# jkulhanek/viewformer

Hardware: AMD Instinct MI355X
Metric: novel views/sec (encode->AR transformer->decode), 128px 6-ctx (higher is better)
Workload: dtype bf16

## Files before the change

include/vf_hip.h:

```cpp
#ifndef VF_HIP_H
#define VF_HIP_H

#include <stddef.h>
#include <stdint.h>

#ifdef __cplusplus
extern "C" {
#endif

#define VF_OK 0
#define VF_ERR_BAD_ARG (-1)
#define VF_ERR_UNSUPPORTED (-2)

int vf_abi_version(void);
size_t vf_sizeof_igemm_args(void);
size_t vf_sizeof_pack_desc(void);
const char* vf_build_arch(void);
int vf_build_flags(void);
const char* vf_build_flag_name(int i);
enum { VF_SEL_ATTN_DMA = 0,
       VF_SEL_GEMM_G256 = 1,
       VF_SEL_LN_BWD_TWO_ROWS = 2,
       VF_SEL_ATTN_Q32 = 3,
       VF_SEL_CONV_X3H_K32 = 4,
// ... 135 lines not shown
                          float* max_logit, void* stream);
int vf_lmhead_score_bf16(const void* h, int h_bf16, int64_t ldh, const void* w_packed, int64_t M, int K, int N, const int32_t* target,
                         int64_t* idx, float* max_logit, float* lse, float* target_logit, float* entropy, void* stream);
int vf_logits_score_f32(const float* logits, int64_t rows, int N, int64_t ld, const int32_t* target, int64_t* idx, float* max_logit,
                        float* lse, float* target_logit, float* entropy, void* stream);
int vf_score_views_f32(const float* target_logit, const float* lse, const float* max_logit, const int64_t* idx, const int32_t* target,
                       int64_t views, int L, float* token_log_prob, float* confidence, float* log_likelihood, float* accuracy, void* stream);
int vf_match_views_f32(const float* logits, int64_t ld, const float* lse, const int64_t* idx, const int32_t* codes, int64_t codes_scene_stride,
                       int64_t B, int64_t M, int64_t P, int L, int V, float* log_likelihood, float* accuracy, void* stream);
int vf_sample_rows_f32(const float* logits, int64_t rows, int N, int64_t ld, float temperature, int top_k, float top_p, uint32_t seed,
                       const int64_t* row_id, int S, int64_t* idx, float* logp, int32_t* kept, float* thr, void* stream);
int vf_sample_views_f32(const float* logp, int64_t views, int L, int S, float* log_likelihood, void* stream);
uint32_t vf_crc32c(const void* data, size_t n, uint32_t crc);
int vf_postprocess_u8(const float* x, uint8_t* out, int64_t n, void* stream);
int vf_resize_u8(const uint8_t* src, uint8_t* dst, int n_img, int Hin, int Win, int Hout, int Wout, int C, int bilinear, void* stream);
size_t vf_image_metrics_workspace_bytes(int n_img, int H, int W, int C);
int vf_image_metrics_u8(const uint8_t* a, const uint8_t* b, int n_img, int H, int W, int C, int64_t* sums, double* ssim, void* workspace,
                        void* stream);
size_t vf_camera_knn_workspace_bytes(int64_t N, int Q, int k);
int vf_camera_knn_f32(const float* db, int64_t N, const float* queries, int Q, int k, float pos_weight, int32_t* idx, float* dist,
                      void* workspace, void* stream);
int vf_codebook_dist_table_f32(const float* E, int D, int K, int64_t ldE, float* table, void* stream);
size_t vf_code_knn_workspace_bytes(int64_t N, int Q, int k);
int vf_code_knn_f32(const int32_t* db, int64_t N, int64_t ld_db, const int32_t* queries, int Q, int64_t ld_q, int t, const float* table,
                    int K, int window, const int32_t* exclude, int k, int32_t* idx, float* dist, void* workspace, void* stream);
int vf_pose_tail_f32(const float* x, int64_t ldx, const float* W, const float* b, float position_multiplier, int64_t views, int L, int K,
                     float* raw, float* tokens, float* cameras, void* stream);

size_t vf_gemm_bf16_packed_elems(int K, int N);
int vf_gemm_bf16_pack(const float* src, void* dst, int K, int N, int64_t sk, int64_t sn, int batch,
                      int64_t src_bstride, void* stream);
typedef struct vf_pack_desc {
    const float* src;
    void* dst;
    int32_t K, N;
    int64_t sk, sn;
} vf_pack_desc;
int vf_gemm_bf16_pack_multi(const vf_pack_desc* descs_device, int n, void* stream);
int vf_gemm_bf16(const vf_igemm_args* args , void* stream);
size_t vf_conv3_bf16_packed_elems(int Cin, int Cout);
int vf_conv3_bf16_pack(const float* w_oihw, void* dst, int Cin, int Cout, void* stream);
int vf_conv3_halo_bf16(const vf_igemm_args* args , void* stream);

int vf_conv3_halo_gn_slots(int Hout, int Wout);
size_t vf_conv3_x6_packed_elems(int Cin, int Cout);
int vf_conv3_x6_pack(const float* w_oihw, void* dst, int Cin, int Cout, void* stream);
int vf_conv3_halo_x6(const vf_igemm_args* args , void* stream);
size_t vf_conv3_x3h_packed_elems(int Cin, int Cout);
int vf_conv3_x3h_pack(const float* w_oihw, void* dst, int Cin, int Cout, void* stream);
int vf_conv3_halo_x3h(const vf_igemm_args* args , void* stream);
size_t vf_gemm_x3h_packed_elems(int K, int N);
int vf_gemm_x3h_pack(const float* src, void* dst, int K, int N, int64_t sk, int64_t sn, void* stream);
int vf_gemm_x3h(const vf_igemm_args* args , void* stream);
size_t vf_gemm_x6_packed_elems(int K, int N);
int vf_gemm_x6_pack(const float* src, void* dst, int K, int N, int64_t sk, int64_t sn, void* stream);
int vf_gemm_x6(const vf_igemm_args* args , void* stream);
int vf_sum_slabs_f32(const float* slabs, int nslabs, int64_t stride, int64_t n, float* dst, int accumulate, void* stream);

int vf_vq_ema_accumulate_f32(const float* z, const int64_t* idx, int64_t M, int D, int Kc, float* counts, float* embed_sum,
                             void* stream);
int vf_vq_ema_update_f32(const float* counts, const float* embed_sum, float* cluster_size_hidden, float* dw_hidden,
                         float* embeddings, int D, int Kc, float decay, float eps, float corr, void* stream);

int vf_gather_transpose_f32(const float* src, float* dst, int n_img, int Hin, int Win, int C, int Hout, int Wout, int stride, int oy,
                            int ox, int64_t ld_dst, void* stream);
size_t vf_conv3_wgrad_x6_rows(int Cin);
int vf_conv3_wgrad_x6(const float* x, const void* dy_packed, float* slabs, int n_img, int Hin, int Win, int Cin, int Hout, int Wout,
                      int Cout, int mode, int splits, void* stream);
int vf_upsample2_bwd_f32(const float* du, float* dx, int n_img, int H, int W, int C, void* stream);
size_t vf_groupnorm_bwd_workspace_bytes(int n_img, int HW, int C, int groups);
int vf_groupnorm_bwd_f32(const float* x, const float* da, const float* mean_c, const float* scale_c, const float* gamma,
                         const float* beta, float* dx, float* chan_sums, int n_img, int HW, int C, int groups, float eps, int swish,
                         int accumulate, void* ws, void* stream);
int vf_softmax_rows_bwd_f32(const float* p, float* dp, int64_t rows, int n, float scale, void* stream);
int vf_l1_loss_partials(int64_t n);
int vf_l1_loss_f32(const float* x, const float* y, float* dy, float* part, int64_t n, float grad_weight, void* stream);

int vf_lpips_scaling_f32(const float* x, float* y, int64_t npix, const float* shift3, const float* scale3, int backward, void* stream);
int vf_relu_f32(float* x, int64_t n, void* stream);
int vf_relu_bwd_f32(float* dy, const float* y, int64_t n, void* stream);
int vf_maxpool2_f32(const float* x, float* y, int n_img, int Hout, int Wout, int C, void* stream);
int vf_maxpool2_bwd_f32(const float* x, const float* dy, float* dx, int n_img, int Hout, int Wout, int C, void* stream);
int vf_lpips_head_blocks(int HW);
int vf_lpips_head_f32(const float* f0, const float* f1, const float* w, float* part, int n_img, int HW, int C, void* stream);
int vf_lpips_head_bwd_f32(const float* f0, const float* f1, const float* w, float* df1, int64_t npix, int C, float gscale,
                          int accumulate, void* stream);

int vf_attn_blockcausal_lse_f32(const float* q, const float* k, const float* v, float* out, float* lse,
                                int B, int H, int T, int L, int ldq, int ldk, int ldv, int ldo,
                                float scale, int skip_masked, int twin_view, float drop_rate, uint32_t drop_seed,
                                uint32_t drop_site, uint32_t drop_plane0, void* stream);
int vf_attn_bwd_prep_f32(const float* dout, const float* out, float* D, int B, int H, int T, int lddo, int ldo, void* stream);
int vf_attn_bwd_f32(const float* q, const float* k, const float* v, const float* dout, const float* lse, const float* D,
                    float* dq, float* dk, float* dv, int B, int H, int T, int L, int ldq, int ldk, int ldv, int lddo,
                    int lddq, int lddk, int lddv, float scale, int twin_view, float drop_rate, uint32_t drop_seed,
                    uint32_t drop_site, uint32_t drop_plane0, void* stream);
int vf_gemm_tn_bf16(const void* x_bf16, int ldx, const void* dy, int dy_is_bf16, int ldy, int M, int K, int N, int splits, float* w_slabs,
                    float* b_slabs, int64_t slab_stride, void* stream);
int vf_attn_blockcausal_bf16_lse(const void* q, const void* k, const void* v, void* out, float* lse, int B, int H, int T, int L,
                                 int ldq, int ldk, int ldv, int ldo, float scale, int twin_view, float drop_rate, uint32_t drop_seed,
                                 uint32_t drop_site, uint32_t drop_plane0, void* stream);
int vf_attn_bwd_prep_bf16(const void* dout, const void* out, float* D, int B, int H, int T, int lddo, int ldo, void* stream);
int vf_attn_bwd_bf16(const void* q, const void* k, const void* v, const void* dout, const float* lse, const float* D, void* dq, void* dk,
                     void* dv, int out_bf16 , int B, int H, int T, int L,
                     int ldq, int ldk, int ldv, int lddo, int lddq, int lddk, int lddv, float scale, int twin_view, float drop_rate,
                     uint32_t drop_seed, uint32_t drop_site, uint32_t drop_plane0, void* stream);
// ... 60 lines not shown
```

viewformer_amd/_lib.py:

```python
import ctypes
import os
from ctypes import c_int, c_int32, c_int64, c_float, c_void_p, c_size_t, c_char_p, POINTER

HERE = os.path.dirname(os.path.abspath(__file__))
LIB_PATH = os.environ.get('VF_HIP_LIB') or os.path.join(HERE, 'libvf_hip.so')


class VfIgemmArgs(ctypes.Structure):
    _fields_ = [
        ('x', c_void_p), ('w_packed', c_void_p), ('bias', c_void_p), ('res', c_void_p), ('out', c_void_p),
        ('pro_mean', c_void_p), ('pro_scale', c_void_p), ('pro_beta', c_void_p),
        ('pro_swish', c_int32), ('pro_rows_per_img', c_int32), ('mode', c_int32), ('epilogue', c_int32),
        ('M', c_int32), ('Cin', c_int32), ('Cout', c_int32),
        ('Hin', c_int32), ('Win', c_int32), ('Hout', c_int32), ('Wout', c_int32),
        ('lda', c_int32), ('ldc', c_int32), ('ldr', c_int32), ('batch', c_int32),
        ('stride_x', c_int64), ('stride_w', c_int64), ('stride_out', c_int64), ('stride_res', c_int64),
        ('gn_part', c_void_p), ('gn_slots', c_int32), ('reserved0', c_int32),
        ('out_aux', c_void_p),
        ('drop_rate', c_float), ('drop_seed', ctypes.c_uint32), ('drop_site', ctypes.c_uint32), ('drop_row0', c_int32),
    ]


SEL_ATTN_DMA, SEL_GEMM_G256, SEL_LN_BWD_TWO_ROWS, SEL_ATTN_Q32 = 0, 1, 2, 3
SEL_CONV_X3H_K32 = 4
# ... 76 lines not shown
    'vf_attn_blockcausal_lse_f32': (c_int, [P, P, P, P, P, c_int, c_int, c_int, c_int, c_int, c_int, c_int, c_int,
                                            c_float, c_int, c_int, c_float, ctypes.c_uint32, ctypes.c_uint32, ctypes.c_uint32, P]),
    'vf_dropout_add_f32': (c_int, [P, P, P, c_int64, c_int, c_int64, c_float, ctypes.c_uint32, ctypes.c_uint32, P]),
    'vf_attn_bwd_prep_f32': (c_int, [P, P, P, c_int, c_int, c_int, c_int, c_int, P]),
    'vf_attn_bwd_f32': (c_int, [P, P, P, P, P, P, P, P, P, c_int, c_int, c_int, c_int, c_int, c_int, c_int, c_int, c_int,
                                c_int, c_int, c_float, c_int, c_float, ctypes.c_uint32, ctypes.c_uint32, ctypes.c_uint32, P]),
    'vf_gemm_tn_bf16': (c_int, [P, c_int, P, c_int, c_int, c_int, c_int, c_int, c_int, P, P, c_int64, P]),
    'vf_attn_blockcausal_bf16_lse': (c_int, [P, P, P, P, P, c_int, c_int, c_int, c_int, c_int, c_int, c_int, c_int, c_float, c_int,
                                             c_float, ctypes.c_uint32, ctypes.c_uint32, ctypes.c_uint32, P]),
    'vf_attn_bwd_prep_bf16': (c_int, [P, P, P, c_int, c_int, c_int, c_int, c_int, P]),
    'vf_attn_bwd_bf16': (c_int, [P, P, P, P, P, P, P, P, P, c_int, c_int, c_int, c_int, c_int, c_int, c_int, c_int, c_int, c_int, c_int, c_int,
                                 c_float, c_int, c_float, ctypes.c_uint32, ctypes.c_uint32, ctypes.c_uint32, P]),
    'vf_attn_spatial_f32': (c_int, [P, P, c_int, c_int, c_int, c_int64, c_int64, c_float, P]),
    'vf_attn_spatial_x3h': (c_int, [P, P, c_int, c_int, c_int, c_int64, c_int64, c_float, P]),
    'vf_softmax_rows_f32': (c_int, [P, c_int64, c_int, c_float, P]),
    'vf_layernorm_f32': (c_int, [P, P, P, P, c_int64, c_int, c_float, P]),
    'vf_layernorm_bf16out_f32': (c_int, [P, P, P, P, c_int64, c_int, c_float, P]),
    'vf_embed_sum_f32': (c_int, [P, P, P, P, P, c_int64, c_int, c_int, c_int, P]),
    'vf_dense_small_k_gelu_f32': (c_int, [P, P, P, P, c_int64, c_int, c_int, c_int, P]),
    'vf_lmhead_argmax_bf16': (c_int, [P, c_int, c_int64, P, c_int64, c_int, c_int, P, P, P]),
    'vf_lmhead_score_bf16': (c_int, [P, c_int, c_int64, P, c_int64, c_int, c_int, P, P, P, P, P, P, P]),
    'vf_logits_score_f32': (c_int, [P, c_int64, c_int, c_int64, P, P, P, P, P, P, P]),
    'vf_score_views_f32': (c_int, [P, P, P, P, P, c_int64, c_int, P, P, P, P, P]),
    'vf_match_views_f32': (c_int, [P, c_int64, P, P, P, c_int64, c_int64, c_int64, c_int64, c_int, c_int, P, P, P]),
    'vf_sample_rows_f32': (c_int, [P, c_int64, c_int, c_int64, c_float, c_int, c_float, ctypes.c_uint32, P, c_int, P, P, P, P, P]),
    'vf_sample_views_f32': (c_int, [P, c_int64, c_int, c_int, P, P]),
    'vf_argmax_rows_f32': (c_int, [P, c_int64, c_int, c_int, P, P]),
    'vf_postprocess_u8': (c_int, [P, P, c_int64, P]),
    'vf_resize_u8': (c_int, [P, P, c_int, c_int, c_int, c_int, c_int, c_int, c_int, P]),
    'vf_image_metrics_workspace_bytes': (c_size_t, [c_int, c_int, c_int, c_int]),
    'vf_image_metrics_u8': (c_int, [P, P, c_int, c_int, c_int, c_int, P, P, P, P]),
    'vf_camera_knn_workspace_bytes': (c_size_t, [c_int64, c_int, c_int]),
    'vf_camera_knn_f32': (c_int, [P, c_int64, P, c_int, c_int, c_float, P, P, P, P]),
    'vf_codebook_dist_table_f32': (c_int, [P, c_int, c_int, c_int64, P, P]),
    'vf_code_knn_workspace_bytes': (c_size_t, [c_int64, c_int, c_int]),
    'vf_code_knn_f32': (c_int, [P, c_int64, c_int64, P, c_int, c_int64, c_int, P, c_int, c_int, P, c_int, P, P, P, P]),
    'vf_pose_tail_f32': (c_int, [P, c_int64, P, P, c_float, c_int64, c_int, c_int, P, P, P, P]),
    'vf_gemm_bf16_packed_elems': (c_size_t, [c_int, c_int]),
    'vf_gemm_bf16_pack': (c_int, [P, P, c_int, c_int, c_int64, c_int64, c_int, c_int64, P]),
    'vf_gemm_bf16_pack_multi': (c_int, [P, c_int, P]),
    'vf_gemm_bf16': (c_int, [POINTER(VfIgemmArgs), P]),
    'vf_conv3_bf16_packed_elems': (c_size_t, [c_int, c_int]),
    'vf_conv3_bf16_pack': (c_int, [P, P, c_int, c_int, P]),
    'vf_conv3_halo_bf16': (c_int, [POINTER(VfIgemmArgs), P]),
    'vf_conv3_x6_packed_elems': (c_size_t, [c_int, c_int]),
    'vf_conv3_x6_pack': (c_int, [P, P, c_int, c_int, P]),
    'vf_conv3_halo_x6': (c_int, [POINTER(VfIgemmArgs), P]),
    'vf_conv3_x3h_packed_elems': (c_size_t, [c_int, c_int]),
    'vf_conv3_x3h_pack': (c_int, [P, P, c_int, c_int, P]),
    'vf_conv3_halo_x3h': (c_int, [POINTER(VfIgemmArgs), P]),
    'vf_gemm_x3h_packed_elems': (c_size_t, [c_int, c_int]),
    'vf_gemm_x3h_pack': (c_int, [P, P, c_int, c_int, c_int64, c_int64, P]),
    'vf_gemm_x3h': (c_int, [POINTER(VfIgemmArgs), P]),
    'vf_gemm_x6_packed_elems': (c_size_t, [c_int, c_int]),
    'vf_gemm_x6_pack': (c_int, [P, P, c_int, c_int, c_int64, c_int64, P]),
    'vf_gemm_x6': (c_int, [POINTER(VfIgemmArgs), P]),
    'vf_sum_slabs_f32': (c_int, [P, c_int, c_int64, c_int64, P, c_int, P]),
    'vf_transpose_f32': (c_int, [P, P, c_int, c_int, c_int64, c_int64, c_int, c_int64, c_int64, P]),
    'vf_transpose_bf16_f32': (c_int, [P, P, c_int, c_int, c_int64, c_int64, c_int, c_int64, c_int64, P]),
    'vf_colsum_workspace_bytes': (c_size_t, [c_int]),
    'vf_colsum_f32': (c_int, [P, P, c_int64, c_int, c_int64, c_int, P, P]),
    'vf_layernorm_bwd_workspace_bytes': (c_size_t, [c_int64, c_int]),
    'vf_layernorm_bwd_f32': (c_int, [P, P, P, P, P, P, c_int64, c_int, c_float, c_int, P, P, c_float, ctypes.c_uint32, ctypes.c_uint32, c_int64, P, P]),
    'vf_gelu_f32': (c_int, [P, P, c_int64, P]),
    'vf_gelu_bf16out_f32': (c_int, [P, P, c_int64, P]),
    'vf_gelu_bwd_bf16out_f32': (c_int, [P, P, P, c_int64, P]),
    'vf_gelu_bwd_f32': (c_int, [P, P, P, c_int64, P]),
    'vf_softmax_mask_f32': (c_int, [P, c_int64, c_int, c_int, c_int, c_float, P]),
    'vf_softmax_mask_bwd_f32': (c_int, [P, P, c_int64, c_int, c_int, c_int, c_float, P]),
    'vf_softmax_ce_f32': (c_int, [P, P, P, P, P, c_int64, c_int, c_float, P]),
    'vf_pose_mse_f32': (c_int, [P, P, P, P, P, P, P, P, c_int64, c_int, c_float, P]),
    'vf_embed_bwd_workspace_bytes': (c_size_t, [c_int, c_int]),
    'vf_embed_bwd_f32': (c_int, [P, P, P, P, P, c_int64, c_int, c_int, c_int, P, P]),
    'vf_dense_small_k_bwd_f32': (c_int, [P, P, P, P, c_int64, c_int, c_int, P]),
    'vf_dense_small_n_f32': (c_int, [P, P, P, P, c_int64, c_int, c_int, c_int64, P]),
    'vf_dense_small_n_wgrad_slabs': (c_int, [c_int64]),
    'vf_dense_small_n_wgrad_f32': (c_int, [P, P, P, P, c_int64, c_int, c_int, c_int64, c_int, P]),
    'vf_adamw_f32': (c_int, [P, P, P, P, c_int64, c_float, c_float, c_float, c_float, c_float, P]),
    'vf_adamw_flat_f32': (c_int, [P, P, P, P, c_int64, P, c_int, c_float, c_float, c_float, c_float, c_float, P]),
    'vf_sizeof_adamw_pack_desc': (c_size_t, []),
    'vf_adamw_pack_check': (c_int, [P, c_int, c_int64]),
    'vf_adamw_flat_pack_f32': (c_int, [P, P, P, P, c_int64, P, c_int, c_float, c_float, c_float, c_float, c_float, P, c_int, P]),
    'vf_axpby_f32': (c_int, [c_float, P, c_float, P, P, c_int64, P]),
    'vf_add_inplace_f32': (c_int, [P, P, c_int64, P]),
    'vf_clip_scratch_floats': (c_int, []),
    'vf_clip_by_norm_f32': (c_int, [P, c_int64, c_float, P, P]),
    'vf_clip_grad_norm_f32': (c_int, [P, c_int64, c_float, P, P]),
}

_lib = None


class VfError(RuntimeError):
    pass


def _bind(path):
    lib = ctypes.CDLL(path)
    for name, (res, args) in EXPORTS.items():
        fn = getattr(lib, name)
        fn.restype = res
        fn.argtypes = args
    return lib


def load_variant(path):
# ... 57 lines not shown
```

viewformer_amd/csrc/gemm_x3h.hip:

```cpp
#include "vf_common.h"
#include "epilogue.h"
#include "../../include/vf_hip.h"

namespace {

typedef _Float16 f16x8 __attribute__((ext_vector_type(8)));
typedef _Float16 f16x4 __attribute__((ext_vector_type(4)));

constexpr int CK = 32;
constexpr int BM = 128, BN = 128;
constexpr int A_LDB = 144;
constexpr int A_BYTES = BM * A_LDB;
constexpr int PLANE_BYTES = 2 * BN * 16;
constexpr int KS_BYTES = 2 * PLANE_BYTES;
constexpr int CHUNK_BYTES = 2 * KS_BYTES;
constexpr int TAIL_BYTES = 16;

__device__ __forceinline__ void split2(float x, _Float16& h, _Float16& l) {
    h = (_Float16)x;
    l = (_Float16)((x - (float)h) * 2048.f);
}

template <bool PRO, bool SWISH, int PIMG = 4>
__global__ __launch_bounds__(256, 2) void gemm_x3h_kernel(vf_igemm_args p) {
    extern __shared__ __attribute__((aligned(16))) unsigned char smem_g[];

    const int tid = threadIdx.x;
    const int lane = tid & 63;
    const int wave = __builtin_amdgcn_readfirstlane(tid >> 6);
    constexpr int MI = 2, NJ = 2;
    const int wave_m = wave >> 1, wave_n = wave & 1;
    const int half = lane >> 5, l31 = lane & 31;

    const int nb = (p.Cout + BN - 1) / BN;
    const unsigned lbid = vf_xcd_bid();
    const int nblk = lbid % nb;
    const int mtile = lbid / nb;
    const float* __restrict__ X = p.x;
    const unsigned char* __restrict__ Wb = reinterpret_cast<const unsigned char*>(p.w_packed) + (size_t)nblk * CHUNK_BYTES;
    const size_t chunk_stride = (size_t)nb * CHUNK_BYTES;
    const int nsplit = p.reserved0 > 1 ? p.reserved0 : 1;
    const int total_chunks = p.Cin / CK;
    const int per = ((total_chunks + nsplit - 1) / nsplit + 1) & ~1;
    const int c0 = min((int)blockIdx.y * per, total_chunks);
    const int nchunks = min(c0 + per, total_chunks);

    const int c4 = tid & 7, r0 = tid >> 3;
    const float* arow[4];
    int aimg[4];
#pragma unroll
    for (int q = 0; q < 4; ++q) {
        int m = mtile * BM + r0 + 32 * q;
// ... 92 lines not shown
            a_park((chunk - c0 + 1) & 1, ks * 2);
            a_park((chunk - c0 + 1) & 1, ks * 2 + 1);
        }
        __builtin_amdgcn_sched_barrier(0);
        __syncthreads();
    };
    for (int chunk = c0; chunk < nchunks; chunk += 2) {
        chunk_body(chunk, bring[0], bring[1]);
        chunk_body(chunk + 1, bring[1], bring[0]);
    }

    const float inv_s = *reinterpret_cast<const float*>(reinterpret_cast<const unsigned char*>(p.w_packed) + (size_t)total_chunks * chunk_stride);
#pragma unroll
    for (int i = 0; i < MI; ++i)
#pragma unroll
        for (int j = 0; j < NJ; ++j)
#pragma unroll
            for (int r = 0; r < 16; ++r) acc[i][j][r] = __builtin_fmaf(accx[i][j][r], 4.8828125e-4f, acc[i][j][r]) * inv_s;
    float* __restrict__ Out = p.out + (size_t)blockIdx.y * p.stride_out;
    const float* __restrict__ Res = p.res;
    const bool full = (mtile * BM + BM <= p.M) && (nblk * BN + BN <= p.Cout);
    const long long ldc = p.ldc, ldr = p.ldr;
    const bool gelu = p.epilogue == VF_EPI_GELU_ERF;
#pragma unroll
    for (int j = 0; j < NJ; ++j) {
        const int n = nblk * BN + wave_n * (32 * NJ) + j * 32 + l31;
        const bool nok = n < p.Cout;
        const float bias = (nok && p.bias) ? p.bias[n] : 0.f;
#pragma unroll
        for (int i = 0; i < MI; ++i) {
            const int m0 = mtile * BM + wave_m * 64 + i * 32 + 4 * half;
            const int nn = nok ? n : 0;
            float* o = Out + (size_t)(m0 < p.M ? m0 : 0) * ldc + nn;
            const float* rs = Res ? Res + (size_t)(m0 < p.M ? m0 : 0) * ldr + nn : nullptr;
            const int rows_left = nok ? p.M - m0 : 0;
            if (full) {
                auto oo = [&](int r) { return (long long)((r & 3) + 8 * (r >> 2)) * ldc; };
                auto ro = [&](int r) { return (long long)((r & 3) + 8 * (r >> 2)) * ldr; };
                if (gelu) {
                    if (Res) vf_store_tile<1, true>(acc[i][j], bias, o, rs, oo, ro);
                    else vf_store_tile<1, false>(acc[i][j], bias, o, rs, oo, ro);
                } else {
                    if (Res) vf_store_tile<0, true>(acc[i][j], bias, o, rs, oo, ro);
                    else vf_store_tile<0, false>(acc[i][j], bias, o, rs, oo, ro);
                }
            } else if (gelu) {
                if (Res) vf_store_tile_ragged<1, true>(acc[i][j], bias, o, rs, ldc, ldr, rows_left);
                else vf_store_tile_ragged<1, false>(acc[i][j], bias, o, rs, ldc, ldr, rows_left);
            } else {
                if (Res) vf_store_tile_ragged<0, true>(acc[i][j], bias, o, rs, ldc, ldr, rows_left);
                else vf_store_tile_ragged<0, false>(acc[i][j], bias, o, rs, ldc, ldr, rows_left);
            }
        }
    }
}


__global__ void absmax_strided_kernel(const float* __restrict__ w, int K, int N, long long sk, long long sn, unsigned* __restrict__ out) {
    float m = 0.f;
    const long long n = (long long)K * N;
    for (long long i = blockIdx.x * (long long)blockDim.x + threadIdx.x; i < n; i += (long long)gridDim.x * blockDim.x)
        m = fmaxf(m, fabsf(w[(i / N) * sk + (i % N) * sn]));
    vf_block_max_atomic(m, out);
}

__global__ void pack_gemm_x3h_kernel(const float* __restrict__ src, _Float16* __restrict__ dst, int K, int N, long long sk,
                                     long long sn, int nb, int nchunks, unsigned char* __restrict__ tail) {
    const float amax = __uint_as_float(*reinterpret_cast<const unsigned*>(tail + 4));
    const int ex = amax > 0.f ? ilogbf(amax) : 13;
    const float S = ldexpf(1.f, 13 - ex);
    if (blockIdx.x == 0 && threadIdx.x == 0) *reinterpret_cast<float*>(tail) = ldexpf(1.f, ex - 13);
    const long long total = (long long)nchunks * nb * CK * BN;
    for (long long idx = blockIdx.x * (long long)blockDim.x + threadIdx.x; idx < total; idx += (long long)gridDim.x * blockDim.x) {
        const int e = (int)(idx & 7);
        long long t = idx >> 3;
        const int nl = (int)(t % BN); t /= BN;
        const int half = (int)(t & 1);
        const int ks = (int)((t >> 1) & 1);
        t >>= 2;
        const int nblk = (int)(t % nb);
        const int chunk = (int)(t / nb);
        const int k = chunk * CK + ks * 16 + half * 8 + e;
        const int n = nblk * BN + nl;
        float v = 0.f;
        if (k < K && n < N) v = src[k * sk + n * sn] * S;
        _Float16 h, l;
        split2(v, h, l);
        const size_t base = ((((size_t)chunk * nb + nblk) * 2 + ks) * 2) * (2 * BN * 8) + ((size_t)half * BN + nl) * 8 + e;
        dst[base] = h;
        dst[base + 2 * BN * 8] = l;
    }
}

template <bool PRO, bool SWISH, int PIMG = 4>
int launch(const vf_igemm_args& a, hipStream_t stream) {
    const size_t smem = (size_t)2 * A_BYTES;
    const int nb = (a.Cout + BN - 1) / BN, mt = (a.M + BM - 1) / BM;
    const int nsplit = a.reserved0 > 1 ? a.reserved0 : 1;
    hipLaunchKernelGGL((gemm_x3h_kernel<PRO, SWISH, PIMG>), dim3((unsigned)(mt * nb), (unsigned)nsplit), dim3(256), smem, stream, a);
    return vf_last_status();
}

}

extern "C" {

size_t vf_gemm_x3h_packed_elems(int K, int N) {
    if (K <= 0 || N <= 0) return 0;
    return (size_t)((K + CK - 1) / CK) * ((N + BN - 1) / BN) * CK * BN * 2 + TAIL_BYTES / 2;
}

int vf_gemm_x3h_pack(const float* src, void* dst, int K, int N, int64_t sk, int64_t sn, void* stream) {
    if (!src || !dst || K <= 0 || N <= 0) return VF_ERR_BAD_ARG;
    const int nb = (N + BN - 1) / BN, nchunks = (K + CK - 1) / CK;
    const long long total = (long long)nchunks * nb * CK * BN;
    unsigned char* tail = reinterpret_cast<unsigned char*>(dst) + (size_t)total * 2 * sizeof(_Float16);
    hipStream_t s = (hipStream_t)stream;
    if (hipMemsetAsync(tail, 0, TAIL_BYTES, s) != hipSuccess) return vf_last_status();
    const long long nw = (long long)K * N;
    hipLaunchKernelGGL(absmax_strided_kernel, dim3((unsigned)((nw + 2047) / 2048 > 128 ? 128 : (nw + 2047) / 2048)), dim3(256), 0, s, src, K,
                       N, (long long)sk, (long long)sn, reinterpret_cast<unsigned*>(tail + 4));
    const int blocks = (int)((total + 255) / 256 > 4096 ? 4096 : (total + 255) / 256);
    hipLaunchKernelGGL(pack_gemm_x3h_kernel, dim3(blocks), dim3(256), 0, s, src, (_Float16*)dst, K, N, (long long)sk, (long long)sn, nb,
                       nchunks, tail);
    return vf_last_status();
}

int vf_gemm_x3h(const vf_igemm_args* args, void* stream) {
    if (!args) return VF_ERR_BAD_ARG;
    const vf_igemm_args& a = *args;
    if (!a.x || !a.w_packed || !a.out || a.M <= 0 || a.Cin <= 0 || a.Cout <= 0) return VF_ERR_BAD_ARG;
    if (a.epilogue != VF_EPI_NONE && a.epilogue != VF_EPI_GELU_ERF) return VF_ERR_UNSUPPORTED;
    if (a.gn_part) return VF_ERR_UNSUPPORTED;
    if (a.drop_rate != 0.f || a.out_aux) return VF_ERR_UNSUPPORTED;
    if (a.mode != VF_MODE_GEMM || a.batch > 1) return VF_ERR_UNSUPPORTED;
    if (a.Cin % 64 != 0) return VF_ERR_UNSUPPORTED;
    if (a.reserved0 > 1 && (a.bias || a.res || a.epilogue != VF_EPI_NONE || a.pro_mean || a.stride_out < (int64_t)a.M * a.ldc))
        return VF_ERR_BAD_ARG;
    if (a.lda < a.Cin || (a.lda & 3) || a.ldc < a.Cout || (a.res && a.ldr < a.Cout)) return VF_ERR_BAD_ARG;
    if ((a.pro_mean || a.pro_scale || a.pro_beta) && !(a.pro_mean && a.pro_scale && a.pro_beta && a.pro_rows_per_img > 0))
        return VF_ERR_BAD_ARG;
    hipStream_t s = (hipStream_t)stream;
    if (!a.pro_mean) return launch<false, false>(a, s);
    if (a.pro_rows_per_img % 128 == 0) return a.pro_swish ? launch<true, true, 1>(a, s) : launch<true, false, 1>(a, s);
    if (a.pro_rows_per_img % 64 == 0) return a.pro_swish ? launch<true, true, 2>(a, s) : launch<true, false, 2>(a, s);
    return a.pro_swish ? launch<true, true>(a, s) : launch<true, false>(a, s);
}

}
```

viewformer_amd/ops.py:

```python
import ctypes
import os

import torch

from . import _lib
from ._lib import VfIgemmArgs, check

MODE_GEMM, MODE_CONV3_S1, MODE_CONV3_S2PAD, MODE_CONV3_UP2 = 0, 1, 2, 3
EPI_NONE, EPI_GELU, EPI_GELU_BWD, EPI_GELU_DUAL = 0, 1, 2, 3


def _stream():
    return ctypes.c_void_p(torch.cuda.current_stream().cuda_stream)


def _p(t):
    if t is None:
        return None
    return ctypes.c_void_p(t.data_ptr())


def _chk(t, dtype=torch.float32, name='tensor'):
    if not t.is_cuda:
        raise _lib.VfError(f'{name} must live on the GPU (no CPU fallback for the hot path)')
# ... 100 lines not shown


def pack_dense_nk_bf16(w, n_rows=None):
    return _pack_dense('bf16', w, True, n_rows)


def pack_conv3_bf16(w_oihw):
    return _pack_conv3('bf16', w_oihw)


def pack_conv3_x6(w_oihw):
    return _pack_conv3('x6', w_oihw)


def pack_conv3_x3h(w_oihw):
    return _pack_conv3('x3h', w_oihw)


def pack_dense_kn_x6(w):
    return _pack_dense('x6', w, False)


def pack_dense_nk_x6(w, n_rows=None):
    return _pack_dense('x6', w, True, n_rows)


def pack_dense_kn_x3h(w):
    return _pack_dense('x3h', w, False)


def pack_dense_nk_x3h(w, n_rows=None):
    return _pack_dense('x3h', w, True, n_rows)


def gemm_x6_splitk(x, w_packed, M, Cin, Cout, dst, splits, lda=None, accumulate=True):
    lib = _lib.load()
    slabs = torch.empty((splits, M, Cout), dtype=torch.float32, device=x.device)
    igemm(x, w_packed, M, Cin, Cout, slabs, lda=lda, x6=True, split_k=splits, stride_out=M * Cout)
    check(lib.vf_sum_slabs_f32(_p(slabs), splits, M * Cout, M * Cout, _p(_f32(dst)), 1 if accumulate else 0, _stream()),
          'vf_sum_slabs_f32')
    return dst


def conv3_x6_supported(mode, Cin, Cout, Hout, Wout):
    if mode not in (MODE_CONV3_S1, MODE_CONV3_UP2, MODE_CONV3_S2PAD) or Cin % 32 or Cout % 128:
        return False
    return (Hout % 8 == 0 and Wout % 16 == 0) or (mode == MODE_CONV3_S1 and Hout == 8 and Wout == 8)


def conv3_x3h_supported(mode, Cin, Cout, Hout, Wout):
    if mode == MODE_CONV3_S2PAD and Hout == 8 and Wout == 8 and Cin % 32 == 0 and Cout % 128 == 0:
        return True
    return conv3_x6_supported(mode, Cin, Cout, Hout, Wout)


ARM_KW = {'f32': {}, 'x6': dict(x6=True), 'x3h': dict(x3h=True), 'bf16': dict(bf16=True)}


def conv3_arm(mode, Cin, Cout, Hout, Wout, activations=False, res=False):
    if not res and conv3_small_cout_supported(mode, Cin, Cout, Hout, Wout):
        return 'small'
    if conv3_x6_supported(mode, Cin, Cout, Hout, Wout):
        return 'x3h' if activations else 'x6'
    return 'f32'


def pack_conv3(arm, w_oihw):
    return {'f32': pack_conv_oihw, 'x6': pack_conv3_x6, 'x3h': pack_conv3_x3h, 'bf16': pack_conv3_bf16}[arm](w_oihw)


def pack_dense_nk_arm(arm, w, n_rows=None):
    return {'f32': pack_dense_nk, 'x6': pack_dense_nk_x6, 'x3h': pack_dense_nk_x3h, 'bf16': pack_dense_nk_bf16}[arm](w, n_rows)


def pack_dense(arm, w, transposed=False, n_rows=None):
    fn = globals()['pack_dense_' + ('nk' if transposed else 'kn') + ('' if arm == 'f32' else '_' + arm)]
    return fn(w) if n_rows is None else fn(w, n_rows=n_rows)


def gemm_bf16_splitk(x, w_packed, M, Cin, Cout, dst, splits, lda=None, accumulate=True):
    lib = _lib.load()
    ks = Cin // splits
    if splits < 1 or ks * splits != Cin or ks % 64:
        raise _lib.VfError(f'gemm_bf16_splitk: Cin = {Cin} does not split into {splits} ranges of whole 64-deep chunks')
    nb = (Cout + 127) // 128
    slabs = torch.empty((splits, M, Cout), dtype=torch.float32, device=x.device)
    igemm(x, w_packed, M, ks, Cout, slabs, lda=Cin if lda is None else lda, bf16=True, batch=splits, stride_x=ks,
          stride_w=(ks // 64) * nb * 64 * 128, stride_out=M * Cout)
    check(lib.vf_sum_slabs_f32(_p(slabs), splits, M * Cout, M * Cout, _p(_f32(dst)), 1 if accumulate else 0, _stream()),
          'vf_sum_slabs_f32')
    return dst


TN_TARGET_WORKGROUPS = 256
TN_TARGET_WORKGROUPS_BESIDE = 192


def gemm_tn_bf16_supported(x, M, K, N):
    return x.dtype == torch.bfloat16 and gemm_tn_bf16_shape_ok(M, K, N)


def gemm_tn_bf16_shape_ok(M, K, N):
    return K % 256 == 0 and N % 256 == 0 and M % 64 == 0 and M * K * 2 < 2 ** 31


def gemm_g256_shape_ok(M, K, N):
# ... 758 lines not shown
```

Baseline: 1131.

## Add persistent 256-wide-N tile kernel for x3h split-precision GEMM

Adds a persistent GEMM kernel for the x3h (split f16 hi/lo) GEMM path. It uses 512 threads, 256-column N blocks and a grid capped at the CU count, and each block loops over tiles. It software-pipelines B buffer loads, A register prefetch, smem parking and an A-fragment ring across chunks and tiles. vf_gemm_x3h now routes eligible shapes (N%256, K%64, no split) to this kernel, which aims to raise data reuse and cut per-tile launch and prologue overhead. In exchange it brings heavier register pressure and a more complex schedule.

Result: no change. 1134 (median of 6 runs) (+0.3%).

```diff
diff --git a/include/vf_hip.h b/include/vf_hip.h
--- a/include/vf_hip.h
+++ b/include/vf_hip.h
@@ -211,6 +211,7 @@
 size_t vf_gemm_x3h_packed_elems(int K, int N);
 int vf_gemm_x3h_pack(const float* src, void* dst, int K, int N, int64_t sk, int64_t sn, void* stream);
 int vf_gemm_x3h(const vf_igemm_args* args , void* stream);
+int vf_gemm_x3h_wide_applies(int M, int K, int N, int nsplit);
 size_t vf_gemm_x6_packed_elems(int K, int N);
 int vf_gemm_x6_pack(const float* src, void* dst, int K, int N, int64_t sk, int64_t sn, void* stream);
 int vf_gemm_x6(const vf_igemm_args* args , void* stream);
diff --git a/viewformer_amd/_lib.py b/viewformer_amd/_lib.py
--- a/viewformer_amd/_lib.py
+++ b/viewformer_amd/_lib.py
@@ -152,6 +152,7 @@
     'vf_gemm_x3h_packed_elems': (c_size_t, [c_int, c_int]),
     'vf_gemm_x3h_pack': (c_int, [P, P, c_int, c_int, c_int64, c_int64, P]),
     'vf_gemm_x3h': (c_int, [POINTER(VfIgemmArgs), P]),
+    'vf_gemm_x3h_wide_applies': (c_int, [c_int, c_int, c_int, c_int]),
     'vf_gemm_x6_packed_elems': (c_size_t, [c_int, c_int]),
     'vf_gemm_x6_pack': (c_int, [P, P, c_int, c_int, c_int64, c_int64, P]),
     'vf_gemm_x6': (c_int, [POINTER(VfIgemmArgs), P]),
diff --git a/viewformer_amd/csrc/gemm_x3h.hip b/viewformer_amd/csrc/gemm_x3h.hip
--- a/viewformer_amd/csrc/gemm_x3h.hip
+++ b/viewformer_amd/csrc/gemm_x3h.hip
@@ -1,3 +1,4 @@
+#include <type_traits>
 #include "vf_common.h"
 #include "epilogue.h"
 #include "../../include/vf_hip.h"
@@ -196,6 +197,227 @@
                 else vf_store_tile_ragged<0, false>(acc[i][j], bias, o, rs, ldc, ldr, rows_left);
             }
         }
+    }
+}
+
+
+constexpr int WBN = 256;
+typedef float f32x4v __attribute__((ext_vector_type(4)));
+
+__device__ __forceinline__ f16x8 wbuf_load(__amdgpu_buffer_rsrc_t r, unsigned voff, unsigned soff) {
+    return __builtin_bit_cast(f16x8, __builtin_amdgcn_raw_buffer_load_b128(r, voff, soff, 0));
+}
+
+template <int EPI, bool HAS_RES>
+__device__ __forceinline__ void wide_store(const f32x4v (&acc)[8][2], const float (&bias)[2], __amdgpu_buffer_rsrc_t o_rs, __amdgpu_buffer_rsrc_t r_rs,
+                                           unsigned ov, unsigned rv, int ldc, int ldr) {
+    float rr[HAS_RES ? 2 : 1][8][4];
+    if (HAS_RES) {
+#pragma unroll
+        for (int ct = 0; ct < 2; ++ct)
+#pragma unroll
+            for (int rt = 0; rt < 8; ++rt)
+#pragma unroll
+                for (int r = 0; r < 4; ++r)
+                    rr[ct][rt][r] = __builtin_bit_cast(float, __builtin_amdgcn_raw_buffer_load_b32(r_rs, rv + ct * 64u + (unsigned)((rt * 16 + 2 * r) * ldr) * 4u, 0u, 0));
+    }
+#pragma unroll
+    for (int ct = 0; ct < 2; ++ct) {
+        float v[8][4];
+#pragma unroll
+        for (int rt = 0; rt < 8; ++rt)
+#pragma unroll
+            for (int r = 0; r < 4; ++r) {
+                float t = acc[rt][ct][r] + bias[ct];
+                if (EPI == 1) t = vf_gelu_erf(t);
+                v[rt][r] = HAS_RES ? t + rr[HAS_RES ? ct : 0][rt][r] : t;
+            }
+#pragma unroll
+        for (int rt = 0; rt < 8; ++rt)
+#pragma unroll
+            for (int r = 0; r < 4; ++r)
+                __builtin_amdgcn_raw_buffer_store_b32(__builtin_bit_cast(unsigned, v[rt][r]), o_rs, ov + ct * 64u + (unsigned)((rt * 16 + 2 * r) * ldc) * 4u, 0u, 0);
+        if (!HAS_RES) __builtin_amdgcn_sched_barrier(0);
+    }
+}
+
+struct WideCursor {
+    int chunk, tile, mt, nblk, img[2];
+};
+
+template <bool PRO, bool SWISH, int PIMG, bool RES>
+__global__ __launch_bounds__(512) void gemm_x3h_wide_kernel(vf_igemm_args p) {
+    extern __shared__ __attribute__((aligned(16))) unsigned char smem_w[];
+    constexpr int RT = 8, CT = 2;
+
+    const int tid = threadIdx.x;
+    const int lane = tid & 63;
+    const int wave = __builtin_amdgcn_readfirstlane(tid >> 6);
+    const int lm = lane & 15, lg = lane >> 4;
+
+    const int nb2 = p.Cout / WBN;
+    const int ntiles = ((p.M + BM - 1) / BM) * nb2;
+    const int G = (int)gridDim.x;
+    const int nchunks = p.Cin / CK;
+    const unsigned chunk_stride = (unsigned)(2 * nb2) * CHUNK_BYTES;
+    const int rpi = PRO ? p.pro_rows_per_img : 1;
+    auto place = [&](WideCursor& c) __attribute__((always_inline)) {
+        c.mt = c.tile / nb2;
+        c.nblk = c.tile - c.mt * nb2;
+        if (PRO) {
+#pragma unroll
+            for (int i = 0; i < PIMG; ++i) c.img[i] = min(c.mt * BM + 64 * i, p.M - 1) / rpi;
+        }
+    };
+    auto advance = [&](WideCursor& c) __attribute__((always_inline)) {
+        if (c.chunk + 1 < nchunks) { ++c.chunk; return; }
+        if (c.tile + G < ntiles) { c.chunk = 0; c.tile += G; place(c); }
+    };
+
+    const int c4 = tid & 7, r0 = tid >> 3;
+    const int c4s = (((c4 >> 1) & 1) * 2 + (c4 >> 2)) * 16 + (c4 & 1) * 8;
+    f32x4 areg[2][2];
+    f32x4 pbeta, pmean[PIMG], pscale[PIMG];
+    auto a_fetch = [&](f32x4 (&dst)[2], const WideCursor& c) {
+        const float* base = p.x + ((size_t)c.mt * BM * p.lda + c.chunk * CK);
+        const int last = p.M - 1 - c.mt * BM;
+#pragma unroll
+        for (int q = 0; q < 2; ++q) dst[q] = *reinterpret_cast<const f32x4*>(base + (unsigned)(min(r0 + 64 * q, last) * p.lda + c4 * 4));
+    };
+    auto p_fetch = [&](const WideCursor& c) __attribute__((always_inline)) {
+        if (!PRO) return;
+        pbeta = *reinterpret_cast<const f32x4*>(p.pro_beta + c.chunk * CK + c4 * 4);
+#pragma unroll
+        for (int i = 0; i < PIMG; ++i) {
+            const size_t po = (size_t)c.img[i] * p.Cin + c.chunk * CK;
+            pmean[i] = *reinterpret_cast<const f32x4*>(p.pro_mean + po + c4 * 4);
+            pscale[i] = *reinterpret_cast<const f32x4*>(p.pro_scale + po + c4 * 4);
+        }
+    };
+    auto a_park = [&](int buf, const f32x4 (&src)[2], int q) {
+        unsigned char* dst = smem_w + buf * A_BYTES + (r0 + 64 * q) * A_LDB + c4s;
+        f16x4 oh, ol;
+#pragma unroll
+        for (int e = 0; e < 4; ++e) {
+            float t = src[q][e];
+            if (PRO) {
+                t = (t - pmean[q * PIMG / 2][e]) * pscale[q * PIMG / 2][e] + pbeta[e];
+                if (SWISH) t = vf_swish_1ulp(t);
+            }
+            _Float16 h, l;
+            split2(t, h, l);
+            oh[e] = h; ol[e] = l;
+        }
+        *reinterpret_cast<f16x4*>(dst) = oh;
+        *reinterpret_cast<f16x4*>(dst + 64) = ol;
+    };
+
+    const int lrow = lm < 4 ? 2 * lm : lm < 12 ? 2 * lm - 7 : 2 * lm - 16;
+    const int a_lane = lrow * A_LDB + (((lg & 1) * 2) + (lg >> 1)) * 16;
+    const __amdgpu_buffer_rsrc_t w_rs = __builtin_amdgcn_make_buffer_rsrc(const_cast<float*>(p.w_packed), 0, 0x7fffffff, 0x00020000);
+    const int b_lane = ((lg >> 1) * 4 + (lg & 1)) * (BN * 16) + ((wave & 3) * 32 + lm) * 16;
+    f16x8 bring[2][4];
+    constexpr int AR = 3;
+    f16x8 aring[AR][2];
+    auto b_load = [&](f16x8 (&dst)[4], const WideCursor& c) {
+        const unsigned soff = (unsigned)c.chunk * chunk_stride + (unsigned)(2 * c.nblk + (wave >> 2)) * CHUNK_BYTES;
+#pragma unroll
+        for (int pl = 0; pl < 2; ++pl)
+#pragma unroll
+            for (int ct = 0; ct < CT; ++ct) dst[pl * 2 + ct] = wbuf_load(w_rs, (unsigned)(b_lane + pl * PLANE_BYTES + ct * 256), soff);
+    };
+    auto a_load = [&](f16x8 (&dst)[2], const unsigned char* img, int rt) {
+        dst[0] = *reinterpret_cast<const f16x8*>(img + a_lane + rt * 16 * A_LDB);
+        dst[1] = *reinterpret_cast<const f16x8*>(img + a_lane + rt * 16 * A_LDB + 64);
+    };
+
+    const float inv_s = *reinterpret_cast<const float*>(reinterpret_cast<const unsigned char*>(p.w_packed) + (size_t)nchunks * chunk_stride);
+    const int pbase = lg == 0 ? 0 : lg == 1 ? 1 : lg == 2 ? 9 : 8;
+    const int ldc = p.ldc, ldr = p.ldr;
+    const bool gelu = p.epilogue == VF_EPI_GELU_ERF;
+
+    WideCursor cc = {0, (int)vf_xcd_bid(), 0, 0, {0, 0}};
+    place(cc);
+    WideCursor cb = cc, cp = cc, cr = cc;
+    b_load(bring[0], cb); advance(cb);
+    p_fetch(cp); advance(cp);
+    a_fetch(areg[0], cr); advance(cr);
+    a_fetch(areg[1], cr); advance(cr);
+    a_park(0, areg[0], 0);
+    a_park(0, areg[0], 1);
+    p_fetch(cp); advance(cp);
+    a_fetch(areg[0], cr); advance(cr);
+    __syncthreads();
+
+    f32x4v acc[RT][CT], accx[RT][CT];
+    auto step_body = [&](auto parity) __attribute__((always_inline)) {
+        constexpr int P0 = decltype(parity)::value;
+        const unsigned char* img = smem_w + P0 * A_BYTES;
+        b_load(bring[P0 ^ 1], cb);
+        advance(cb);
+        a_load(aring[0], img, 0);
+        a_load(aring[1], img, 1);
+        const f16x8 (&B)[4] = bring[P0];
+#pragma unroll
+        for (int rt = 0; rt < RT; ++rt) {
+            if (rt + AR - 1 < RT) a_load(aring[(rt + AR - 1) % AR], img, rt + AR - 1);
+            if (rt == 1) a_park(P0 ^ 1, areg[P0 ^ 1], 0);
+            if (rt == 2) a_park(P0 ^ 1, areg[P0 ^ 1], 1);
+            if (rt == 3) {
+                p_fetch(cp); advance(cp);
+                a_fetch(areg[P0 ^ 1], cr); advance(cr);
+            }
+            const f16x8 ah = aring[rt % AR][0], al = aring[rt % AR][1];
+            accx[rt][0] = __builtin_amdgcn_mfma_f32_16x16x32_f16(al, B[0], accx[rt][0], 0, 0, 0);
+            accx[rt][1] = __builtin_amdgcn_mfma_f32_16x16x32_f16(al, B[1], accx[rt][1], 0, 0, 0);
+            acc[rt][0] = __builtin_amdgcn_mfma_f32_16x16x32_f16(ah, B[0], acc[rt][0], 0, 0, 0);
+            acc[rt][1] = __builtin_amdgcn_mfma_f32_16x16x32_f16(ah, B[1], acc[rt][1], 0, 0, 0);
+            accx[rt][0] = __builtin_amdgcn_mfma_f32_16x16x32_f16(ah, B[2], accx[rt][0], 0, 0, 0);
+            accx[rt][1] = __builtin_amdgcn_mfma_f32_16x16x32_f16(ah, B[3], accx[rt][1], 0, 0, 0);
+            __builtin_amdgcn_sched_barrier(0);
+        }
+        __syncthreads();
+    };
+    auto tile_steps = [&]() __attribute__((always_inline)) {
+#pragma unroll
+        for (int i = 0; i < RT; ++i)
+#pragma unroll
+            for (int j = 0; j < CT; ++j)
+#pragma unroll
+                for (int r = 0; r < 4; ++r) { acc[i][j][r] = 0.f; accx[i][j][r] = 0.f; }
+        step_body(std::integral_constant<int, 0>{});
+        step_body(std::integral_constant<int, 1>{});
+        for (int chunk = 2; chunk < nchunks; chunk += 2) {
+            step_body(std::integral_constant<int, 0>{});
+            step_body(std::integral_constant<int, 1>{});
+        }
+    };
+    auto tile_store = [&]() __attribute__((always_inline)) {
+#pragma unroll
+        for (int rt = 0; rt < RT; ++rt)
+#pragma unroll
+            for (int ct = 0; ct < CT; ++ct)
+#pragma unroll
+                for (int r = 0; r < 4; ++r) acc[rt][ct][r] = __builtin_fmaf(accx[rt][ct][r], 4.8828125e-4f, acc[rt][ct][r]) * inv_s;
+        __builtin_amdgcn_sched_barrier(0);
+        const int rows = min(BM, p.M - cc.mt * BM);
+        const __amdgpu_buffer_rsrc_t o_rs =
+            __builtin_amdgcn_make_buffer_rsrc(p.out + (size_t)cc.mt * BM * ldc, 0, ((rows - 1) * ldc + p.Cout) * 4, 0x00020000);
+        const __amdgpu_buffer_rsrc_t r_rs = __builtin_amdgcn_make_buffer_rsrc(RES ? const_cast<float*>(p.res) + (size_t)cc.mt * BM * ldr : p.out, 0,
+                                                                              RES ? ((rows - 1) * ldr + p.Cout) * 4 : 0, 0x00020000);
+        const int n0 = cc.nblk * WBN + wave * 32 + lm;
+        const float bias2[CT] = {p.bias ? p.bias[n0] : 0.f, p.bias ? p.bias[n0 + 16] : 0.f};
+        const unsigned ov = (unsigned)(pbase * ldc + n0) * 4u, rv = (unsigned)(pbase * ldr + n0) * 4u;
+        if (gelu) wide_store<1, RES>(acc, bias2, o_rs, r_rs, ov, rv, ldc, ldr);
+        else wide_store<0, RES>(acc, bias2, o_rs, r_rs, ov, rv, ldc, ldr);
+    };
+    tile_steps();
+    tile_store();
+    while (cc.tile + G < ntiles) {
+        cc.tile += G;
+        place(cc);
+        tile_steps();
+        tile_store();
     }
 }
 
@@ -245,9 +467,67 @@
     return vf_last_status();
 }
 
+bool wide_applies(int M, int K, int N, int nsplit) {
+    return M > 0 && K > 0 && N > 0 && N % WBN == 0 && K % 64 == 0 && nsplit <= 1 && (long long)K * N < (1ll << 29);
+}
+
+int wide_cus() {
+    static int n = 0;
+    if (!n) {
+        int d = 0, c = 0;
+        n = (hipGetDevice(&d) == hipSuccess && hipDeviceGetAttribute(&c, hipDeviceAttributeMultiprocessorCount, d) == hipSuccess && c > 0) ? c : 256;
+    }
+    return n;
+}
+
+template <bool PRO, bool SWISH, int PIMG>
+int launch_wide(const vf_igemm_args& a, hipStream_t stream) {
+    const size_t smem = (size_t)2 * A_BYTES;
+    const int ntiles = ((a.M + BM - 1) / BM) * (a.Cout / WBN);
+    const dim3 grid((unsigned)(ntiles < wide_cus() ? ntiles : wide_cus()));
+    if constexpr (!PRO) {
+        if (a.res) {
+            hipLaunchKernelGGL((gemm_x3h_wide_kernel<false, false, 1, true>), grid, dim3(512), smem, stream, a);
+            return vf_last_status();
+        }
+    }
+    hipLaunchKernelGGL((gemm_x3h_wide_kernel<PRO, SWISH, PIMG, false>), grid, dim3(512), smem, stream, a);
+    return vf_last_status();
+}
+
+bool wide_takes(const vf_igemm_args& a) {
+    return wide_applies(a.M, a.Cin, a.Cout, a.reserved0) && a.lda < (1 << 22) && a.ldc < (1 << 22) && (!a.res || a.ldr < (1 << 22)) &&
+           (!a.pro_mean || (a.pro_rows_per_img % 64 == 0 && !a.res));
+}
+
+int dispatch_wide(const vf_igemm_args& a, hipStream_t s) {
+    if (!a.pro_mean) return launch_wide<false, false, 1>(a, s);
+    if (a.pro_rows_per_img % 128 == 0) return a.pro_swish ? launch_wide<true, true, 1>(a, s) : launch_wide<true, false, 1>(a, s);
+    return a.pro_swish ? launch_wide<true, true, 2>(a, s) : launch_wide<true, false, 2>(a, s);
+}
+
+int check_args(const vf_igemm_args* args) {
+    if (!args) return VF_ERR_BAD_ARG;
+    const vf_igemm_args& a = *args;
+    if (!a.x || !a.w_packed || !a.out || a.M <= 0 || a.Cin <= 0 || a.Cout <= 0) return VF_ERR_BAD_ARG;
+    if (a.epilogue != VF_EPI_NONE && a.epilogue != VF_EPI_GELU_ERF) return VF_ERR_UNSUPPORTED;
+    if (a.gn_part) return VF_ERR_UNSUPPORTED;
+    if (a.drop_rate != 0.f || a.out_aux) return VF_ERR_UNSUPPORTED;
+    if (a.mode != VF_MODE_GEMM || a.batch > 1) return VF_ERR_UNSUPPORTED;
+    if (a.Cin % 64 != 0) return VF_ERR_UNSUPPORTED;
+    if (a.reserved0 > 1 && (a.bias || a.res || a.epilogue != VF_EPI_NONE || a.pro_mean || a.stride_out < (int64_t)a.M * a.ldc))
+        return VF_ERR_BAD_ARG;
+    if (a.lda < a.Cin || (a.lda & 3) || a.ldc < a.Cout || (a.res && a.ldr < a.Cout)) return VF_ERR_BAD_ARG;
+    if ((a.pro_mean || a.pro_scale || a.pro_beta) && !(a.pro_mean && a.pro_scale && a.pro_beta && a.pro_rows_per_img > 0))
+        return VF_ERR_BAD_ARG;
+    return VF_OK;
+}
+
 }
 
 extern "C" {
+
+int vf_gemm_x3h_wide_applies(int M, int K, int N, int nsplit) { return wide_applies(M, K, N, nsplit) ? 1 : 0; }
 
 size_t vf_gemm_x3h_packed_elems(int K, int N) {
     if (K <= 0 || N <= 0) return 0;
@@ -271,20 +551,11 @@
 }
 
 int vf_gemm_x3h(const vf_igemm_args* args, void* stream) {
-    if (!args) return VF_ERR_BAD_ARG;
+    const int rc = check_args(args);
+    if (rc != VF_OK) return rc;
     const vf_igemm_args& a = *args;
-    if (!a.x || !a.w_packed || !a.out || a.M <= 0 || a.Cin <= 0 || a.Cout <= 0) return VF_ERR_BAD_ARG;
-    if (a.epilogue != VF_EPI_NONE && a.epilogue != VF_EPI_GELU_ERF) return VF_ERR_UNSUPPORTED;
-    if (a.gn_part) return VF_ERR_UNSUPPORTED;
-    if (a.drop_rate != 0.f || a.out_aux) return VF_ERR_UNSUPPORTED;
-    if (a.mode != VF_MODE_GEMM || a.batch > 1) return VF_ERR_UNSUPPORTED;
-    if (a.Cin % 64 != 0) return VF_ERR_UNSUPPORTED;
-    if (a.reserved0 > 1 && (a.bias || a.res || a.epilogue != VF_EPI_NONE || a.pro_mean || a.stride_out < (int64_t)a.M * a.ldc))
-        return VF_ERR_BAD_ARG;
-    if (a.lda < a.Cin || (a.lda & 3) || a.ldc < a.Cout || (a.res && a.ldr < a.Cout)) return VF_ERR_BAD_ARG;
-    if ((a.pro_mean || a.pro_scale || a.pro_beta) && !(a.pro_mean && a.pro_scale && a.pro_beta && a.pro_rows_per_img > 0))
-        return VF_ERR_BAD_ARG;
     hipStream_t s = (hipStream_t)stream;
+    if (wide_takes(a)) return dispatch_wide(a, s);
     if (!a.pro_mean) return launch<false, false>(a, s);
     if (a.pro_rows_per_img % 128 == 0) return a.pro_swish ? launch<true, true, 1>(a, s) : launch<true, false, 1>(a, s);
     if (a.pro_rows_per_img % 64 == 0) return a.pro_swish ? launch<true, true, 2>(a, s) : launch<true, false, 2>(a, s);
diff --git a/viewformer_amd/ops.py b/viewformer_amd/ops.py
--- a/viewformer_amd/ops.py
+++ b/viewformer_amd/ops.py
@@ -176,6 +176,10 @@
     if mode == MODE_CONV3_S2PAD and Hout == 8 and Wout == 8 and Cin % 32 == 0 and Cout % 128 == 0:
         return True
     return conv3_x6_supported(mode, Cin, Cout, Hout, Wout)
+
+
+def gemm_x3h_wide_applies(M, K, N, split_k=0):
+    return bool(_lib.load().vf_gemm_x3h_wide_applies(M, K, N, split_k))
 
 
 ARM_KW = {'f32': {}, 'x6': dict(x6=True), 'x3h': dict(x3h=True), 'bf16': dict(bf16=True)}
```
